# ForeverFancy/GVFDiffusion

Measured on AMD Instinct MI355X. Metric: 4D frames/sec (800x800x24f, 256k Gaussians) + DiT denoise steps/sec, higher is better.
Workload: dtype f32; 1 GPU; BASELINE configs[1]: single-GPU HIP rasteriser, one 4D sample per step = 24 frames x 800x800, 262144 Gaussians + per-frame deltas (fused activations), SH degree 2, mip 2D filter, white bg; gaussians=262144, resolution=800, sh_degree=2, parallelism=sample-sharded x1, samples_in_flight=2

## Files before the change

gvfdiffusion_amd/csrc/rast_blend.hip:

```cpp
#include "rast_common.h"

namespace {


__global__ __launch_bounds__(1024) void blend_order_kernel(const uint2* __restrict__ ranges, int ntiles, uint32_t* __restrict__ order) {
    __shared__ uint32_t hist[64];
    const int f = blockIdx.x, t = threadIdx.x;
    const uint2* r = ranges + (size_t)f * ntiles;
    if (t < 64) hist[t] = 0u;
    __syncthreads();
    for (int tile = t; tile < ntiles; tile += 1024) {
        const uint32_t n = r[tile].y - r[tile].x;
        atomicAdd(&hist[63u - min(63u, n >> 5)], 1u);
    }
    __syncthreads();
    const bool reorder = hist[0] != 0u;
    __syncthreads();
    if (!reorder) {
        for (int tile = t; tile < ntiles; tile += 1024) order[(size_t)f * ntiles + tile] = (uint32_t)tile;
        return;
    }
    if (t == 0) {
        uint32_t run = 0u;
        for (int c = 0; c < 64; ++c) { const uint32_t h = hist[c]; hist[c] = run; run += h; }
    }
    __syncthreads();
    for (int tile = t; tile < ntiles; tile += 1024) {
        const uint32_t n = r[tile].y - r[tile].x;
        order[(size_t)f * ntiles + atomicAdd(&hist[63u - min(63u, n >> 5)], 1u)] = (uint32_t)tile;
    }
}

#ifdef BLEND_TIMING
__device__ unsigned long long* g_blend_buf;
__device__ unsigned long long g_blend_cap;
extern "C" int gvf_debug_blend_timing(unsigned long long* device_buf, unsigned long long rows) {
    if (hipMemcpyToSymbol(HIP_SYMBOL(g_blend_buf), &device_buf, sizeof(device_buf)) != hipSuccess) return 1;
    if (hipMemcpyToSymbol(HIP_SYMBOL(g_blend_cap), &rows, sizeof(rows)) != hipSuccess) return 1;
    return 0;
}
#define BT_DECL unsigned long long bt_acc[12] = {}; unsigned long long bt_last = __builtin_amdgcn_s_memtime(); const unsigned long long bt_first = bt_last;
#define BT(i) do { const unsigned long long n_ = __builtin_amdgcn_s_memtime(); bt_acc[i] += n_ - bt_last; bt_last = n_; } while (0)
#define BT_VMWAIT() asm volatile("s_waitcnt vmcnt(0)" ::: "memory")
#else
#define BT_DECL
#define BT(i) do { } while (0)
#define BT_VMWAIT() do { } while (0)
#endif

#ifdef BLEND_CONSUMED
__device__ unsigned long long g_blend_cons[4][5];
extern "C" int gvf_debug_blend_consumed(unsigned long long* out12, int reset) {
    if (out12 && hipMemcpyFromSymbol(out12, HIP_SYMBOL(g_blend_cons), sizeof(g_blend_cons)) != hipSuccess) return 1;
    if (reset) { unsigned long long z[20] = {}; if (hipMemcpyToSymbol(HIP_SYMBOL(g_blend_cons), z, sizeof(z)) != hipSuccess) return 1; }
    return 0;
}
#endif


template <bool DEPTH>
__global__ __launch_bounds__(BLEND_THREADS) void blend_kernel(
    int P, int H, int W, int gx, int gy, float bg0, float bg1, float bg2, const uint2* __restrict__ ranges,
    const uint32_t* __restrict__ point_list, const float4* __restrict__ splats,
    const float* __restrict__ subpixel_offset, float* __restrict__ out_color,
    float* __restrict__ out_alpha, float* __restrict__ out_depth,
    const uint32_t* __restrict__ tile_order ,
    const uint32_t* __restrict__ rec_of ,
    unsigned char* __restrict__ out_u8 ) {
    __shared__ float4 sA[BLEND_THREADS];
    __shared__ float4 sB[BLEND_THREADS];
    __shared__ float4 sC[BLEND_THREADS];
    __shared__ unsigned char sMask[BLEND_THREADS];
    __shared__ unsigned sList[4][BLEND_THREADS];

    const int t = threadIdx.x, lane = t & 63, wave = t >> 6;
    const int f = blockIdx.y;
    const int tile = tile_order != nullptr ? (int)tile_order[(size_t)f * gridDim.x + blockIdx.x] : (int)blockIdx.x;
    const int tx = tile % gx, ty = tile / gx;
    const int px = tx * TILE + (wave & 1) * 8 + (lane & 7), py = ty * TILE + (wave >> 1) * 8 + (lane >> 3);
    const bool inside = px < W && py < H;
    const size_t pid = (size_t)py * W + px;
    float pxf = (float)px, pyf = (float)py;
    if (subpixel_offset != nullptr && inside) { pxf += subpixel_offset[2 * pid]; pyf += subpixel_offset[2 * pid + 1]; }

    const uint2 rng = ranges[(size_t)f * gx * gy + tile];
    const size_t gbase = (size_t)f * P;
    const int rounds = (int)((rng.y - rng.x + BLEND_THREADS - 1) / BLEND_THREADS);
    int todo = (int)(rng.y - rng.x);
    const uint64_t lt_mask = (1ull << lane) - 1ull;

    const float pxr = pxf - (float)(tx * TILE), pyr = pyf - (float)(ty * TILE);
    unsigned long long done_m = __builtin_amdgcn_ballot_w64(!inside);
    float T = 1.0f, C0 = 0.f, C1 = 0.f, C2 = 0.f, Dacc = 0.f;

    BT_DECL
#ifdef BLEND_CONSUMED
    int rounds_done = rounds;
#endif
    for (int r = 0; r < rounds; ++r, todo -= BLEND_THREADS) {
        BT(6);
#ifdef BLEND_CONSUMED
        if (r > 0 && __syncthreads_and(done_m == ~0ull)) { rounds_done = r; break; }
#else
        if (r > 0 && __syncthreads_and(done_m == ~0ull)) break;
#endif
        BT(0);
#ifdef BLEND_TIMING
        uint32_t id_ = 0;
        if (t < todo) id_ = point_list[rng.x + (uint32_t)r * BLEND_THREADS + t];
        if (t < todo && rec_of != nullptr) id_ = rec_of[id_];
        BT_VMWAIT(); BT(1);
        float4 a_ = {}, b_ = {}, c_ = {};
        if (t < todo) { const float4* rec = splats + 4 * (gbase + id_); a_ = rec[0]; c_ = rec[2]; b_ = rec[1]; }
        BT_VMWAIT(); BT(2);
        bt_acc[7] += 1;
#endif
        if (t < todo) {
#ifdef BLEND_TIMING
            const float4 a = a_, b = b_, c = c_;
#else
            uint32_t id = point_list[rng.x + (uint32_t)r * BLEND_THREADS + t];
            if (rec_of != nullptr) id = rec_of[id];
            const float4* rec = splats + 4 * (gbase + id);
            const float4 a = rec[0];
            const float4 c = rec[2];
            const float4 b = rec[1];
#endif
            const SplatChol ch = splat_cholesky(a.x, a.y, a.z, a.w, b.x, (float)(tx * TILE), (float)(ty * TILE));
            sA[t] = make_float4(ch.l11, ch.l12, ch.l22, ch.c1);
            sB[t] = make_float4(ch.c2, ch.ok ? __builtin_amdgcn_logf(b.y) : -__builtin_inff(), b.z, b.w);
            sC[t] = make_float4(c.x, c.y, 0.f, 0.f);
            sMask[t] = (unsigned char)quadrant_mask(a.x, a.y, a.z, a.w, b.x, b.y, c.z, (float)(tx * TILE), (float)(ty * TILE), subpixel_offset != nullptr);
#ifdef BLEND_CONSUMED
            {
                const unsigned n_ = rng.y - rng.x;
                const int cls_ = n_ <= 2048u ? 0 : n_ <= 4096u ? 1 : n_ <= 16384u ? 2 : 3;
                if (sMask[t] == 0) atomicAdd(&g_blend_cons[cls_][3], 1ull);
                atomicAdd(&g_blend_cons[cls_][4], (unsigned long long)__popc((unsigned)sMask[t]));
            }
#endif
        }
        BT(3);
        __syncthreads();
        BT(4);
        const int cnt = min(BLEND_THREADS, todo);
        if (done_m == ~0ull) continue;
        int n_w = 0;
#pragma unroll
        for (int k = 0; k < BLEND_THREADS / GVF_WAVE; ++k) {
            const int idx = k * GVF_WAVE + lane;
            const bool hit = idx < cnt && ((sMask[idx] >> wave) & 1u);
            const uint64_t bal = __ballot(hit);
            if (hit) sList[wave][n_w + __popcll(bal & lt_mask)] = (unsigned)idx * 16u;
            n_w += __popcll(bal);
        }
        __builtin_amdgcn_wave_barrier();
        BT(5);
#ifdef BLEND_TIMING
        bt_acc[8] += n_w;
#endif
#define GVF_BLEND_STEP(J)                                                                              \
        {                                                                                              \
            const float4 a = *reinterpret_cast<const float4*>(reinterpret_cast<const unsigned char*>(sA) + (J));          \
            const float4 b = *reinterpret_cast<const float4*>(reinterpret_cast<const unsigned char*>(sB) + (J));          \
            const float4 c4_ = *reinterpret_cast<const float4*>(reinterpret_cast<const unsigned char*>(sC) + (J));        \
            const float2 c = DEPTH ? make_float2(c4_.x, c4_.y) : make_float2(c4_.x, 0.f);              \
            const float nlog = splat_neg_exponent(a.x, a.y, a.z, a.w, b.x, pxr, pyr, b.y);    \
            const float alpha = fminf(0.99f, __builtin_amdgcn_exp2f(-nlog));                           \
            const float w_raw = alpha * T;                                                             \
            const float test_T = T - w_raw;         \
                              \
            const unsigned long long ok_m = __builtin_amdgcn_ballot_w64(!(alpha < 1.0f / 255.0f)) & ~done_m;   \
            const unsigned long long stop_m = ok_m & __builtin_amdgcn_ballot_w64(test_T < 0.0001f);    \
            done_m |= stop_m;                                                                          \
            const bool acc = __builtin_amdgcn_inverse_ballot_w64(ok_m ^ stop_m);                       \
            const float wgt = acc ? w_raw : 0.0f;                                                      \
            C0 = __builtin_fmaf(b.z, wgt, C0);                                                         \
            C1 = __builtin_fmaf(b.w, wgt, C1);                                                         \
            C2 = __builtin_fmaf(c.x, wgt, C2);                                                         \
            if (DEPTH) Dacc = __builtin_fmaf(c.y, wgt, Dacc);                                          \
            T = acc ? test_T : T;                                                                      \
        }
        int jj = 0;
        for (; jj + 3 < n_w; jj += 4) {
            if (done_m == ~0ull) break;
            const unsigned j0 = sList[wave][jj], j1 = sList[wave][jj + 1], j2 = sList[wave][jj + 2], j3 = sList[wave][jj + 3];
            GVF_BLEND_STEP(j0)
            GVF_BLEND_STEP(j1)
            __builtin_amdgcn_sched_barrier(0);
            GVF_BLEND_STEP(j2)
            GVF_BLEND_STEP(j3)
        }
        for (; jj < n_w; ++jj) {
            if (done_m == ~0ull) break;
            const unsigned j0 = sList[wave][jj];
            GVF_BLEND_STEP(j0)
        }
#undef GVF_BLEND_STEP
    }
#ifdef BLEND_CONSUMED
    if (t == 0) {
        const unsigned n = rng.y - rng.x, used = min(n, (unsigned)rounds_done * BLEND_THREADS);
        const int cls = n <= 2048u ? 0 : n <= 4096u ? 1 : n <= 16384u ? 2 : 3;
        atomicAdd(&g_blend_cons[cls][0], 1ull); atomicAdd(&g_blend_cons[cls][1], (unsigned long long)n); atomicAdd(&g_blend_cons[cls][2], (unsigned long long)used);
    }
#endif
    if (inside) {
        const size_t hw = (size_t)H * W;
        const float r0 = __builtin_fmaf(T, bg0, C0), r1 = __builtin_fmaf(T, bg1, C1), r2 = __builtin_fmaf(T, bg2, C2);
        if (out_u8 != nullptr) {
            unsigned char* ob = out_u8 + (size_t)f * 3 * hw;
            ob[0 * hw + pid] = (unsigned char)(fminf(fmaxf(r0, 0.f), 1.f) * 255.0f);
            ob[1 * hw + pid] = (unsigned char)(fminf(fmaxf(r1, 0.f), 1.f) * 255.0f);
            ob[2 * hw + pid] = (unsigned char)(fminf(fmaxf(r2, 0.f), 1.f) * 255.0f);
        } else {
            float* oc = out_color + (size_t)f * 3 * hw;
            oc[0 * hw + pid] = r0;
            oc[1 * hw + pid] = r1;
            oc[2 * hw + pid] = r2;
        }
        if (out_alpha != nullptr) out_alpha[(size_t)f * hw + pid] = 1.0f - T;
        if (out_depth != nullptr) out_depth[(size_t)f * hw + pid] = Dacc;
    }
#ifdef BLEND_TIMING
    BT(6);
    BT_VMWAIT(); BT(11);
    bt_acc[9] = 1; bt_acc[10] = bt_last - bt_first;
    const unsigned long long wid = ((unsigned long long)f * gridDim.x + tile) * 4 + wave;
    if (lane == 0 && g_blend_buf != nullptr && wid < g_blend_cap)
        for (int i = 0; i < 12; ++i) g_blend_buf[wid * 12 + i] = bt_acc[i];
#endif
}

__global__ __launch_bounds__(256) void rgb_to_u8_kernel(const float4* __restrict__ src, uchar4* __restrict__ dst,
                                                        long long n4, const float* __restrict__ tail_src,
                                                        unsigned char* __restrict__ tail_dst, int tail) {
    for (long long i = blockIdx.x * (long long)blockDim.x + threadIdx.x; i < n4; i += (long long)gridDim.x * blockDim.x) {
        const float4 v = src[i];
        uchar4 o;
        o.x = (unsigned char)(fminf(fmaxf(v.x, 0.f), 1.f) * 255.0f);
        o.y = (unsigned char)(fminf(fmaxf(v.y, 0.f), 1.f) * 255.0f);
        o.z = (unsigned char)(fminf(fmaxf(v.z, 0.f), 1.f) * 255.0f);
        o.w = (unsigned char)(fminf(fmaxf(v.w, 0.f), 1.f) * 255.0f);
        dst[i] = o;
    }
    if (blockIdx.x == 0 && (int)threadIdx.x < tail)
        tail_dst[threadIdx.x] = (unsigned char)(fminf(fmaxf(tail_src[threadIdx.x], 0.f), 1.f) * 255.0f);
}

}

int gvf_rast::launch_blend(hipStream_t stream, const GvfRastSettings& st, int P, int F, const uint2* ranges, const uint32_t* point_list,
                           const float4* splats, const float* subpixel_offset, float* out_color, float* out_alpha, float* out_depth,
                           unsigned char* out_u8, const uint32_t* rec_of, uint32_t* tile_order, hipEvent_t ordered) {
    const int H = st.image_height, W = st.image_width;
    const int gx = (W + TILE - 1) / TILE, gy = (H + TILE - 1) / TILE, ntiles = gx * gy;
    if (tile_order != nullptr) hipLaunchKernelGGL(blend_order_kernel, dim3(F), dim3(1024), 0, stream, ranges, ntiles, tile_order);
    if (ordered != nullptr) (void)hipEventRecord(ordered, stream);
    hipLaunchKernelGGL(out_depth != nullptr ? blend_kernel<true> : blend_kernel<false>, dim3(ntiles, F), dim3(BLEND_THREADS), 0, stream, P, H, W,
                       gx, gy, st.bg[0], st.bg[1], st.bg[2], ranges, point_list, splats, subpixel_offset, out_color, out_alpha, out_depth,
                       tile_order, rec_of, out_u8);
    GVF_CHECK_LAUNCH();
    return GVF_OK;
}

extern "C" int gvf_rgb_to_u8(const float* rgb, uint8_t* out, int64_t n, void* stream) {
    if (n < 0) return GVF_EINVAL;
    if (n == 0) return GVF_OK;
    if (!rgb || !out || (((uintptr_t)rgb) & 15) || (((uintptr_t)out) & 3)) return GVF_EINVAL;
    (void)hipGetLastError();
    const long long n4 = n / 4;
    long long blocks = (n4 + 255) / 256;
    if (blocks < 1) blocks = 1;
    if (blocks > 8192) blocks = 8192;
    hipLaunchKernelGGL(rgb_to_u8_kernel, dim3((unsigned)blocks), dim3(256), 0, (hipStream_t)stream,
                       reinterpret_cast<const float4*>(rgb), reinterpret_cast<uchar4*>(out), n4, rgb + n4 * 4,
                       out + n4 * 4, (int)(n - n4 * 4));
    GVF_CHECK_LAUNCH();
    return GVF_OK;
}
```

gvfdiffusion_amd/csrc/rast_common.h:

```cpp
#pragma once
#include "gvf_common.h"
#include "../../include/gvf_rast.h"
#include "rast_plan.h"
using namespace gvf_rast;
static_assert(WAVE == GVF_WAVE, "rast_plan.h sizes its grids for this wave width");

namespace {

constexpr int BLEND_THREADS = TILE * TILE;
constexpr int MAX_SH_COEFFS = 16;
constexpr float CONIC_K1 = -0.7213475204444817f;
constexpr float CONIC_K2 = -1.4426950408889634f;
constexpr float CONIC_IK1 = -1.3862943611198906f;
constexpr float CONIC_IK2 = -0.6931471805599453f;
struct SplatChol { float l11, l12, l22, c1, c2; bool ok; };
__device__ __forceinline__ SplatChol splat_cholesky(float x, float y, float ap, float bp, float cp, float tile_x0, float tile_y0) {
    SplatChol r;
    const float m11 = -ap, m12 = -0.5f * bp, m22 = -cp;
    const float il = __builtin_amdgcn_rsqf(m11);
    r.l11 = m11 * il;
    r.l12 = m12 * il;
    const float d = m22 - r.l12 * r.l12;
    r.l22 = __builtin_amdgcn_sqrtf(d);
    r.ok = m11 > 0.0f && d > 0.0f && m11 < __builtin_inff() && d < __builtin_inff();
    if (!r.ok) { r.l11 = 0.f; r.l12 = 0.f; r.l22 = 0.f; }
    const float xr = x - tile_x0, yr = y - tile_y0;
    r.c1 = r.ok ? __builtin_fmaf(r.l11, xr, r.l12 * yr) : 0.f;
    r.c2 = r.ok ? r.l22 * yr : 0.f;
    return r;
}
__device__ __forceinline__ float splat_neg_exponent(float l11, float l12, float l22, float c1, float c2, float px, float py, float lo = 0.0f) {
    const float s1 = __builtin_fmaf(-l11, px, __builtin_fmaf(-l12, py, c1));
    const float s2 = __builtin_fmaf(-l22, py, c2);
    return __builtin_fmaf(s2, s2, __builtin_fmaf(s1, s1, -lo));
}

__constant__ float SH_C0 = 0.28209479177387814f;
__constant__ float SH_C1 = 0.4886025119029199f;
__constant__ float SH_C2[5] = {1.0925484305920792f, -1.0925484305920792f, 0.31539156525252005f,
                               -1.0925484305920792f, 0.5462742152960396f};
__constant__ float SH_C3[7] = {-0.5900435899266435f, 2.890611442640554f, -0.4570457994644658f,
                               0.3731763325901154f, -0.4570457994644658f, 1.445305721320277f,
                               -0.5900435899266435f};

__device__ __forceinline__ float act_expf(float x) {
    if (x != x) return x;
    if (x > 88.72283f) return __builtin_inff();
    if (x < -103.97208f) return 0.0f;
    const float kf = x * 1.44269502f + (x < 0.0f ? -0.5f : 0.5f);
    const int k = (int)kf;
    const float t = (float)k;
    float r = __builtin_fmaf(t, -0.693145751953125f, x);
    r = __builtin_fmaf(t, -1.42860677e-6f, r);
    float p = 1.98412698e-4f;
    p = __builtin_fmaf(p, r, 1.38888889e-3f);
    p = __builtin_fmaf(p, r, 8.33333377e-3f);
    p = __builtin_fmaf(p, r, 4.16666679e-2f);
    p = __builtin_fmaf(p, r, 1.66666672e-1f);
    p = __builtin_fmaf(p, r, 0.5f);
    p = __builtin_fmaf(p, r, 1.0f);
    p = __builtin_fmaf(p, r, 1.0f);
    const int k1 = k / 2, k2 = k - k1;
    return (p * __uint_as_float((uint32_t)(k1 + 127) << 23)) * __uint_as_float((uint32_t)(k2 + 127) << 23);
}
__device__ __forceinline__ float act_log1pf(float y) {
    if (!(y >= 5.9604645e-8f)) return y;
    if (y > 3.4028235e38f) return y;
    int k = 0;
    float c = 0.0f, f = y;
    if (y >= 0.41421354f) {
        const float u = 1.0f + y;
        uint32_t iu = __float_as_uint(u) + (0x3f800000u - 0x3f3504f3u);
        k = (int)(iu >> 23) - 127;
        if (k < 25) c = (k >= 2 ? 1.0f - (u - y) : y - (u - 1.0f)) / u;
        iu = (iu & 0x007fffffu) + 0x3f3504f3u;
        f = __uint_as_float(iu) - 1.0f;
    }
    const float s = f / (2.0f + f);
    const float z = s * s, w = z * z;
    const float t1 = w * (0.40000972152f + w * 0.24279078841f);
    const float t2 = z * (0.66666662693f + w * 0.28498786688f);
    const float R = t2 + t1;
    const float hfsq = (0.5f * f) * f;
    const float dk = (float)k;
    float acc = s * (hfsq + R);
    acc = acc + (dk * 9.0580006145e-6f + c);
    acc = acc - hfsq;
    acc = acc + f;
    return acc + dk * 6.9313812256e-1f;
}
__device__ __forceinline__ float act_scale(float x, const GvfGaussianActivation& a) {
    float s = a.scaling_activation == 0 ? act_expf(x) : (x > 20.0f ? x : act_log1pf(act_expf(x)));
    return sqrtf(s * s + a.min_kernel_size * a.min_kernel_size);
}

struct ActGaussian {
    float p[3], s[3], q[4], op, drgb[3];
};

struct ActRaw {
    float p[3], s[3], q[4], op;
};
__device__ __forceinline__ ActRaw activate_raw(int i, const GvfGaussianActivation& a,
                                               const float* __restrict__ xyz_raw,
                                               const float* __restrict__ scaling_raw,
                                               const float* __restrict__ rotation_raw,
                                               const float* __restrict__ opacity_raw) {
    ActRaw r;
#pragma unroll
    for (int k = 0; k < 3; ++k) r.p[k] = xyz_raw[3 * (size_t)i + k] * a.aabb[3 + k] + a.aabb[k];
#pragma unroll
    for (int k = 0; k < 3; ++k) r.s[k] = scaling_raw[3 * (size_t)i + k] + a.scale_bias;
#pragma unroll
    for (int k = 0; k < 4; ++k) r.q[k] = rotation_raw[4 * (size_t)i + k] + (k == 0 ? 1.0f : 0.0f);
    r.op = opacity_raw[i] + a.opacity_bias;
    return r;
}
__device__ __forceinline__ ActGaussian activate_finish(const ActRaw& r, const GvfGaussianActivation& a, const float (&dl)[14], bool d) {
    ActGaussian g;
#pragma unroll
    for (int k = 0; k < 3; ++k) g.p[k] = d ? r.p[k] + dl[k] : r.p[k];
#pragma unroll
    for (int k = 0; k < 3; ++k) {
        float x = r.s[k];
        if (d) x = x + dl[3 + k];
        g.s[k] = act_scale(x, a);
    }
    float q[4];
#pragma unroll
    for (int k = 0; k < 4; ++k) {
        q[k] = r.q[k];
        if (d) q[k] = q[k] + dl[6 + k];
    }
    float n = sqrtf(q[0] * q[0] + q[1] * q[1] + q[2] * q[2] + q[3] * q[3]);
    n = fmaxf(n, 1e-12f);
#pragma unroll
    for (int k = 0; k < 4; ++k) g.q[k] = q[k] / n;
    float x = r.op;
    if (d) x = x + dl[13];
    g.op = 1.0f / (1.0f + act_expf(-x));
    g.drgb[0] = dl[10]; g.drgb[1] = dl[11]; g.drgb[2] = dl[12];
    return g;
}
__device__ __forceinline__ ActGaussian activate_vals(int i, const GvfGaussianActivation& a,
                                                     const float* __restrict__ xyz_raw,
                                                     const float* __restrict__ scaling_raw,
                                                     const float* __restrict__ rotation_raw,
                                                     const float* __restrict__ opacity_raw,
                                                     const float (&dl)[14], bool d) {
    return activate_finish(activate_raw(i, a, xyz_raw, scaling_raw, rotation_raw, opacity_raw), a, dl, d);
}
__device__ __forceinline__ ActGaussian activate_one(int i, const GvfGaussianActivation& a,
                                                    const float* __restrict__ xyz_raw,
                                                    const float* __restrict__ scaling_raw,
                                                    const float* __restrict__ rotation_raw,
                                                    const float* __restrict__ opacity_raw,
                                                    const float* __restrict__ d ) {
    float dl[14];
#pragma unroll
    for (int k = 0; k < 14; ++k) dl[k] = d ? d[k] : 0.0f;
    return activate_vals(i, a, xyz_raw, scaling_raw, rotation_raw, opacity_raw, dl, d != nullptr);
}

__device__ __forceinline__ void xform43(const float* m, const float* p, float* o) {
    o[0] = m[0] * p[0] + m[4] * p[1] + m[8] * p[2] + m[12];
    o[1] = m[1] * p[0] + m[5] * p[1] + m[9] * p[2] + m[13];
    o[2] = m[2] * p[0] + m[6] * p[1] + m[10] * p[2] + m[14];
}
__device__ __forceinline__ void xform44(const float* m, const float* p, float* o) {
    o[0] = m[0] * p[0] + m[4] * p[1] + m[8] * p[2] + m[12];
    o[1] = m[1] * p[0] + m[5] * p[1] + m[9] * p[2] + m[13];
    o[2] = m[2] * p[0] + m[6] * p[1] + m[10] * p[2] + m[14];
    o[3] = m[3] * p[0] + m[7] * p[1] + m[11] * p[2] + m[15];
}

__device__ __forceinline__ void cov3d_from_scale_rot(const float* s, float mod, const float* q, float* c6) {
    float sx = mod * s[0], sy = mod * s[1], sz = mod * s[2];
    float r = q[0], x = q[1], y = q[2], z = q[3];
    float R00 = 1.f - 2.f * (y * y + z * z), R01 = 2.f * (x * y - r * z), R02 = 2.f * (x * z + r * y);
    float R10 = 2.f * (x * y + r * z), R11 = 1.f - 2.f * (x * x + z * z), R12 = 2.f * (y * z - r * x);
    float R20 = 2.f * (x * z - r * y), R21 = 2.f * (y * z + r * x), R22 = 1.f - 2.f * (x * x + y * y);
    float L00 = R00 * sx, L01 = R01 * sy, L02 = R02 * sz;
    float L10 = R10 * sx, L11 = R11 * sy, L12 = R12 * sz;
    float L20 = R20 * sx, L21 = R21 * sy, L22 = R22 * sz;
    c6[0] = L00 * L00 + L01 * L01 + L02 * L02;
    c6[1] = L00 * L10 + L01 * L11 + L02 * L12;
    c6[2] = L00 * L20 + L01 * L21 + L02 * L22;
    c6[3] = L10 * L10 + L11 * L11 + L12 * L12;
    c6[4] = L10 * L20 + L11 * L21 + L12 * L22;
    c6[5] = L20 * L20 + L21 * L21 + L22 * L22;
}

__device__ __forceinline__ void sh_to_rgb(int deg, const float* sh, const float* dadd, const float* p,
                                          const float* cam, float* rgb) {
    float dx = p[0] - cam[0], dy = p[1] - cam[1], dz = p[2] - cam[2];
    float len = sqrtf(dx * dx + dy * dy + dz * dz);
    float x = dx / len, y = dy / len, z = dz / len;
#pragma unroll
    for (int c = 0; c < 3; ++c) {
        const float da = dadd[c];
        float res = SH_C0 * (sh[0 * 3 + c] + da);
        if (deg > 0) {
            res = res - SH_C1 * y * (sh[1 * 3 + c] + da) + SH_C1 * z * (sh[2 * 3 + c] + da) -
                  SH_C1 * x * (sh[3 * 3 + c] + da);
            if (deg > 1) {
                float xx = x * x, yy = y * y, zz = z * z, xy = x * y, yz = y * z, xz = x * z;
                res = res + SH_C2[0] * xy * (sh[4 * 3 + c] + da) + SH_C2[1] * yz * (sh[5 * 3 + c] + da) +
                      SH_C2[2] * (2.0f * zz - xx - yy) * (sh[6 * 3 + c] + da) +
                      SH_C2[3] * xz * (sh[7 * 3 + c] + da) + SH_C2[4] * (xx - yy) * (sh[8 * 3 + c] + da);
                if (deg > 2) {
                    res = res + SH_C3[0] * y * (3.0f * xx - yy) * (sh[9 * 3 + c] + da) +
                          SH_C3[1] * xy * z * (sh[10 * 3 + c] + da) +
                          SH_C3[2] * y * (4.0f * zz - xx - yy) * (sh[11 * 3 + c] + da) +
                          SH_C3[3] * z * (2.0f * zz - 3.0f * xx - 3.0f * yy) * (sh[12 * 3 + c] + da) +
                          SH_C3[4] * x * (4.0f * zz - xx - yy) * (sh[13 * 3 + c] + da) +
                          SH_C3[5] * z * (xx - yy) * (sh[14 * 3 + c] + da) +
                          SH_C3[6] * x * (xx - 3.0f * yy) * (sh[15 * 3 + c] + da);
                }
            }
        }
        res += 0.5f;
        rgb[c] = res < 0.f ? 0.f : res;
    }
}

struct TileRect { int x0, y0, x1, y1; };
__device__ __forceinline__ TileRect get_rect(float px, float py, float radius, int gx, int gy) {
    TileRect r;
    r.x0 = min(gx, max(0, (int)((px - radius) / (float)TILE)));
    r.y0 = min(gy, max(0, (int)((py - radius) / (float)TILE)));
    r.x1 = min(gx, max(0, (int)((px + radius + (float)(TILE - 1)) / (float)TILE)));
    r.y1 = min(gy, max(0, (int)((py + radius + (float)(TILE - 1)) / (float)TILE)));
    return r;
}

#ifndef GVF_SORT_SMALL_N
#define GVF_SORT_SMALL_N 1536
#endif
constexpr int SORT_SMALL_N = GVF_SORT_SMALL_N;
static_assert(SORT_SMALL_N == 1536 || SORT_SMALL_N == 2048, "register class of the per-tile sort: 6 or 8 keys per thread");
constexpr int SORT_LARGE_N = 16384;
constexpr int SORT_LARGE_BLOCKS = 256, SORT_HUGE_BLOCKS = 64;
constexpr int SORT_MEDIUM_N = 4096, SORT_MEDIUM_BLOCKS = 768;

__device__ __forceinline__ float edge_max(float qa, float qb, float qc, float kv, float fixed, float lo, float hi) {
    const float t = fminf(fmaxf(kv * fixed, lo), hi);
    return __builtin_fmaf(__builtin_fmaf(qc, t, qb * fixed), t, (qa * fixed) * fixed);
}
__device__ __forceinline__ unsigned quadrant_mask(float x, float y, float ap, float bp, float cp, float op, float hx,
                                                  float tile_x0, float tile_y0, bool no_cull) {
    if (hx < 0.0f) return 0u;
    if (no_cull || !(hx < __builtin_inff())) return 0xFu;
    const float lim = -(__log2f(255.0f * op) + 0.02f);
    const float kx = -0.5f * bp * __builtin_amdgcn_rcpf(cp), ky = -0.5f * bp * __builtin_amdgcn_rcpf(ap);
    const float xr = x - tile_x0, yr = y - tile_y0;
    unsigned m = 0u;
#pragma unroll
    for (int q = 0; q < 4; ++q) {
        const float ox = (float)((q & 1) * 8), oy = (float)((q >> 1) * 8);
        const float dxl = xr - (ox + 7.0f), dxh = xr - ox, dyl = yr - (oy + 7.0f), dyh = yr - oy;
        const bool inside = dxl <= 0.0f && dxh >= 0.0f && dyl <= 0.0f && dyh >= 0.0f;
        float e = edge_max(ap, bp, cp, kx, dxl, dyl, dyh);
        e = fmaxf(e, edge_max(ap, bp, cp, kx, dxh, dyl, dyh));
        e = fmaxf(e, edge_max(cp, bp, ap, ky, dyl, dxl, dxh));
        e = fmaxf(e, edge_max(cp, bp, ap, ky, dyh, dxl, dxh));
        m |= (inside || e >= lim) ? (1u << q) : 0u;
    }
    return m;
}

constexpr int BWD_ACC = 10;

}

namespace gvf_rast {

struct Workspace {
    GvfRastFrame* frames;
    float4* splats;
    uint32_t* tiles_touched; int32_t* radii;
    uint32_t* block_sums; uint32_t* frame_base; uint32_t* total;
    uint64_t* keys; uint64_t* keys_alt; uint32_t* vals; uint32_t* vals_alt; uint32_t* ids;
    uint2* ranges; uint32_t* cls;
    uint32_t* tile_count; uint32_t* cursor;
    uint32_t* partial;
    uint32_t* order; uint32_t* order_alt; uint32_t* mhist; uint32_t* mm;
    uint4* binrec;
    void* sort_tmp; size_t sort_tmp_bytes;
    size_t bytes; bool ok;
};

Workspace carve(void* ws, size_t bytes, int P, int F, int H, int W, int64_t max_rendered);

struct RastCall {
    const GvfRastSettings* st; const GvfRastFrame* frames_host; int F, P, M;
    bool fused; const GvfGaussianActivation* act;
    const float *a0, *a1, *a2, *a3, *sh, *colors_precomp, *cov3D_precomp, *delta; int n_delta;
    const float* subpixel_offset;
    int64_t max_rendered;
    int32_t* out_radii; uint32_t* out_num_rendered;
};

inline void prof_mark(hipStream_t s, const hipEvent_t* marks, int k) {
    if (marks != nullptr) (void)hipEventRecord(marks[k], s);
}

int upload_frames(hipStream_t stream, const RastCall& c, const RastPlan& plan, const Workspace& w);
int front_end_bucket(hipStream_t stream, const RastCall& c, const RastPlan& plan, const Workspace& w, const hipEvent_t* marks);
int front_end_radix(hipStream_t stream, const RastCall& c, const RastPlan& plan, const Workspace& w, const hipEvent_t* marks,
                    uint64_t** keys_sorted, uint32_t** vals_by_tile);

int launch_tile_sort(hipStream_t stream, const uint2* ranges, uint64_t* keys, const uint32_t* vals, uint32_t* ids, uint32_t* cls,
                     uint32_t nseg, int cls_state);
int tile_sort_set_lds_limit();

int launch_blend(hipStream_t stream, const GvfRastSettings& st, int P, int F, const uint2* ranges, const uint32_t* point_list,
                 const float4* splats, const float* subpixel_offset, float* out_color, float* out_alpha, float* out_depth,
                 unsigned char* out_u8, const uint32_t* rec_of, uint32_t* tile_order, hipEvent_t ordered);
}
using namespace gvf_rast;
```

Measured before the change: 22420 frames/s.

## Unroll blend loop by eight, branchless activations, cheaper quadrant edge test

Adds an 8-wide unrolled blend loop ahead of the 4-wide one, with scheduling barriers between pairs of steps. Rewrites act_expf and act_log1pf as branch-free clamp-and-select code, gating the log1p range split on a wave ballot to cut divergence. The quadrant culling now evaluates two edges instead of four, picking the nearer x and y edge. The narrower edge test can change which quadrants are kept, and the larger unroll raises register pressure.

```diff
diff --git a/gvfdiffusion_amd/csrc/rast_blend.hip b/gvfdiffusion_amd/csrc/rast_blend.hip
--- a/gvfdiffusion_amd/csrc/rast_blend.hip
+++ b/gvfdiffusion_amd/csrc/rast_blend.hip
@@ -182,6 +182,22 @@
             T = acc ? test_T : T;                                                                      \
         }
         int jj = 0;
+        for (; jj + 7 < n_w; jj += 8) {
+            if (done_m == ~0ull) break;
+            const unsigned j0 = sList[wave][jj], j1 = sList[wave][jj + 1], j2 = sList[wave][jj + 2], j3 = sList[wave][jj + 3];
+            GVF_BLEND_STEP(j0)
+            GVF_BLEND_STEP(j1)
+            __builtin_amdgcn_sched_barrier(0);
+            GVF_BLEND_STEP(j2)
+            GVF_BLEND_STEP(j3)
+            __builtin_amdgcn_sched_barrier(0);
+            const unsigned j4 = sList[wave][jj + 4], j5 = sList[wave][jj + 5], j6 = sList[wave][jj + 6], j7 = sList[wave][jj + 7];
+            GVF_BLEND_STEP(j4)
+            GVF_BLEND_STEP(j5)
+            __builtin_amdgcn_sched_barrier(0);
+            GVF_BLEND_STEP(j6)
+            GVF_BLEND_STEP(j7)
+        }
         for (; jj + 3 < n_w; jj += 4) {
             if (done_m == ~0ull) break;
             const unsigned j0 = sList[wave][jj], j1 = sList[wave][jj + 1], j2 = sList[wave][jj + 2], j3 = sList[wave][jj + 3];
diff --git a/gvfdiffusion_amd/csrc/rast_common.h b/gvfdiffusion_amd/csrc/rast_common.h
--- a/gvfdiffusion_amd/csrc/rast_common.h
+++ b/gvfdiffusion_amd/csrc/rast_common.h
@@ -44,13 +44,11 @@
                                -0.5900435899266435f};
 
 __device__ __forceinline__ float act_expf(float x) {
-    if (x != x) return x;
-    if (x > 88.72283f) return __builtin_inff();
-    if (x < -103.97208f) return 0.0f;
-    const float kf = x * 1.44269502f + (x < 0.0f ? -0.5f : 0.5f);
+    const float xc = fminf(fmaxf(x, -103.97208f), 88.72283f);
+    const float kf = xc * 1.44269502f + (xc < 0.0f ? -0.5f : 0.5f);
     const int k = (int)kf;
     const float t = (float)k;
-    float r = __builtin_fmaf(t, -0.693145751953125f, x);
+    float r = __builtin_fmaf(t, -0.693145751953125f, xc);
     r = __builtin_fmaf(t, -1.42860677e-6f, r);
     float p = 1.98412698e-4f;
     p = __builtin_fmaf(p, r, 1.38888889e-3f);
@@ -61,20 +59,24 @@
     p = __builtin_fmaf(p, r, 1.0f);
     p = __builtin_fmaf(p, r, 1.0f);
     const int k1 = k / 2, k2 = k - k1;
-    return (p * __uint_as_float((uint32_t)(k1 + 127) << 23)) * __uint_as_float((uint32_t)(k2 + 127) << 23);
+    float e = (p * __uint_as_float((uint32_t)(k1 + 127) << 23)) * __uint_as_float((uint32_t)(k2 + 127) << 23);
+    e = x < -103.97208f ? 0.0f : e;
+    e = x > 88.72283f ? __builtin_inff() : e;
+    return x != x ? x : e;
 }
 __device__ __forceinline__ float act_log1pf(float y) {
-    if (!(y >= 5.9604645e-8f)) return y;
-    if (y > 3.4028235e38f) return y;
+    const bool split = y >= 0.41421354f;
     int k = 0;
     float c = 0.0f, f = y;
-    if (y >= 0.41421354f) {
+    if (__builtin_amdgcn_ballot_w64(split) != 0ull) {
         const float u = 1.0f + y;
         uint32_t iu = __float_as_uint(u) + (0x3f800000u - 0x3f3504f3u);
-        k = (int)(iu >> 23) - 127;
-        if (k < 25) c = (k >= 2 ? 1.0f - (u - y) : y - (u - 1.0f)) / u;
+        const int ks = (int)(iu >> 23) - 127;
+        const float cs = (ks >= 2 ? 1.0f - (u - y) : y - (u - 1.0f)) / u;
         iu = (iu & 0x007fffffu) + 0x3f3504f3u;
-        f = __uint_as_float(iu) - 1.0f;
+        k = split ? ks : 0;
+        c = split && ks < 25 ? cs : 0.0f;
+        f = split ? __uint_as_float(iu) - 1.0f : y;
     }
     const float s = f / (2.0f + f);
     const float z = s * s, w = z * z;
@@ -87,10 +89,13 @@
     acc = acc + (dk * 9.0580006145e-6f + c);
     acc = acc - hfsq;
     acc = acc + f;
-    return acc + dk * 6.9313812256e-1f;
+    acc = acc + dk * 6.9313812256e-1f;
+    return (!(y >= 5.9604645e-8f) || y > 3.4028235e38f) ? y : acc;
 }
 __device__ __forceinline__ float act_scale(float x, const GvfGaussianActivation& a) {
-    float s = a.scaling_activation == 0 ? act_expf(x) : (x > 20.0f ? x : act_log1pf(act_expf(x)));
+    float s;
+    if (a.scaling_activation == 0) s = act_expf(x);
+    else { s = act_log1pf(act_expf(x)); s = x > 20.0f ? x : s; }
     return sqrtf(s * s + a.min_kernel_size * a.min_kernel_size);
 }
 
@@ -260,10 +265,8 @@
         const float ox = (float)((q & 1) * 8), oy = (float)((q >> 1) * 8);
         const float dxl = xr - (ox + 7.0f), dxh = xr - ox, dyl = yr - (oy + 7.0f), dyh = yr - oy;
         const bool inside = dxl <= 0.0f && dxh >= 0.0f && dyl <= 0.0f && dyh >= 0.0f;
-        float e = edge_max(ap, bp, cp, kx, dxl, dyl, dyh);
-        e = fmaxf(e, edge_max(ap, bp, cp, kx, dxh, dyl, dyh));
-        e = fmaxf(e, edge_max(cp, bp, ap, ky, dyl, dxl, dxh));
-        e = fmaxf(e, edge_max(cp, bp, ap, ky, dyh, dxl, dxh));
+        const float fx = dxl > 0.0f ? dxl : dxh, fy = dyl > 0.0f ? dyl : dyh;
+        const float e = fmaxf(edge_max(ap, bp, cp, kx, fx, dyl, dyh), edge_max(cp, bp, ap, ky, fy, dxl, dxh));
         m |= (inside || e >= lim) ? (1u << q) : 0u;
     }
     return m;
```

New measurement: 22350 frames/s. Within noise of the previous version (-0.3%).
